# HpWang-whu/YOHO

Measured on AMD Instinct MI355X. Metric: keypoints/sec (5000 kp x60 rot desc+YOHO-O), higher is better.
Workload: dtype fp16x2 split (2^-22-accurate products, fp32 accumulate); 1 GPU

## Files before the change

yoho_amd/csrc/api.hip:

```cpp
#include "common.h"
#include <cstdarg>
#include <cstdio>
#include <cstring>
#include <cstdlib>
#include <cmath>
#include <vector>

namespace yoho {

static thread_local char g_err[512] = "";

void set_error(const char* fmt, ...) {
    va_list ap;
    va_start(ap, fmt);
    vsnprintf(g_err, sizeof(g_err), fmt, ap);
    va_end(ap);
}

void clear_error() { g_err[0] = 0; }

int hip_fail(hipError_t e, const char* what, const char* file, int line) {
    set_error("HIP error %d (%s) at %s:%d: %s", (int)e, hipGetErrorString(e), file, line, what);
    return YOHO_EHIP;
}
// ... 297 lines not shown
        const std::vector<int>* lists[3] = {&all, &two, &one};
        for (int cfg = 0; cfg < 3; ++cfg) {
            const std::vector<int>& gl = *lists[cfg];
            int* ug = &unitg[cfg * 64];
            for (size_t k = 0; k < gl.size(); ++k) ug[k] = gl[k];
            for (int tp = 0; tp < 7; ++tp)
                for (int u = 0; u < 32; ++u)
                    for (int gs = 0; gs < 2; ++gs)
                        for (int h = 0; h < 2; ++h) {
                            int g = ug[2 * u + gs];
                            if (g < 0) g = ug[2 * u];
                            int tap = 2 * tp + h;
                            if (tap >= NTAP) tap = 2 * tp;
                            slab4[(cfg * 7 + tp) * 32 + u] |= (g < 0 ? 0 : (int)N[g * NTAP + tap]) << (8 * (2 * gs + h));
                        }
        }
        if ((rc = upload_slot_tables16(slab4.data(), unitg.data(), c->tabs)) || (rc = gconv16_init())) { delete c; return rc; }
    }
    c->gconv_mode = 4;
    c->partII_mode = 2;
    {
        auto is = [](const char* name, const char* val) { const char* e = std::getenv(name); return e && std::strcmp(e, val) == 0; };
        auto num = [](const char* name) { const char* e = std::getenv(name); return e ? std::atoi(e) : 0; };
        c->env.partII_tail_staged = is("YOHO_PARTII_TAIL", "staged");
        c->env.transfer_staged = is("YOHO_TRANSFER", "staged");
        c->env.xf_steal = !is("YOHO_XF_STEAL", "0");
        c->env.nn_splits = num("YOHO_NN_SPLITS");
        c->env.fcgf_f32 = is("YOHO_FCGF", "f32");
        c->env.fcgf_full_maps = is("YOHO_FCGF_MAPS", "full");
        c->env.fcgf_norm_staged = is("YOHO_FCGF_NORM", "staged");
        c->env.fcgf_heads_staged = is("YOHO_FCGF_HEADS", "staged");
        if (const char* e = std::getenv("YOHO_WS_LIMIT_MB")) c->env.ws_limit_mb = std::atoll(e);
        if (is("YOHO_PARTII_L1", "3")) c->env.partII_l1_variant = FG_TILE256_W8;
    }
    if (const char* m = std::getenv("YOHO_FCGF_CELLS")) c->fcgf_cell_sort = std::atoi(m);
    if (const char* m = std::getenv("YOHO_FCGF_SORT")) c->fcgf_parity_sort = std::strcmp(m, "0") == 0 ? 0 : 1;
    if (const char* m = std::getenv("YOHO_FCGF_COORDS")) c->fcgf_hash_coords = std::strcmp(m, "hash") == 0 ? 1 : 0;
    if (const char* m = std::getenv("YOHO_NN")) c->nn_prefilter = std::strcmp(m, "brute") == 0 ? 0 : 1;
    if (const char* m = std::getenv("YOHO_PARTII")) c->partII_mode = std::strcmp(m, "f32") == 0 ? 0 : (std::strcmp(m, "fp16x2") == 0 ? 2 : (std::strcmp(m, "cgemm") == 0 ? 3 : (std::strcmp(m, "cgemm8") == 0 ? 4 : 1)));
    if (const char* m = std::getenv("YOHO_PARTI_CHUNK")) {
        int ck = 0, ns = 1;
        if (std::sscanf(m, "%dx%d", &ck, &ns) >= 1 && ck >= 0 && (ns == 1 || ns == 2)) { c->partI_chunk = (ck + 255) / 256 * 256; c->partI_streams = ns; }
    }
    if (const char* m = std::getenv("YOHO_GCONV")) c->gconv_mode = std::strcmp(m, "f32") == 0 ? 0 : (std::strcmp(m, "bf16x3") == 0 ? 1 : (std::strcmp(m, "fp16x2") == 0 ? 3 : (std::strcmp(m, "fgemm") == 0 ? 4 : (std::strcmp(m, "fgemm256") == 0 ? 5 : (std::strcmp(m, "fgemm128") == 0 ? 6 : (std::strcmp(m, "fgemm8") == 0 ? 7 : 2))))));
    c->fb = new FourierBasis();
    if ((rc = build_fourier(N, P, *c->fb))) { delete c->fb; delete c; return rc; }
    {
        std::vector<float> fpad(2 * 64 * 64, 0.f);
        for (int s = 0; s < G; ++s)
            for (int g = 0; g < G; ++g) {
                fpad[s * 64 + g] = (float)c->fb->F[s * G + g];
                fpad[64 * 64 + g * 64 + s] = (float)c->fb->F[s * G + g];
            }
        if ((rc = upload(fpad.data(), fpad.size() * sizeof(float), (void**)&c->dFpad)) || (rc = gft_init()) || (rc = fgemm_init()) || (rc = gft16_init())) { delete c->fb; delete c; return rc; }
        std::vector<unsigned short> f16;
        build_gft16_frags(*c->fb, f16);
        if ((rc = upload(f16.data(), f16.size() * sizeof(unsigned short), &c->dF16))) { delete c->fb; delete c; return rc; }
        hipDeviceProp_t prop;
        if (hipGetDeviceProperties(&prop, device) == hipSuccess && prop.multiProcessorCount > 0) c->nCU = prop.multiProcessorCount;
    }
    HIPCHK(hipMalloc((void**)&c->d_rflag, 4 * sizeof(int)));
    HIPCHK(hipMemset(c->d_rflag, 0, 4 * sizeof(int)));
    HIPCHK(hipMalloc((void**)&c->d_amax, 12 * sizeof(unsigned)));
    HIPCHK(hipMemset(c->d_amax, 0, 12 * sizeof(unsigned)));
    {
        for (int g = 0; g < G; ++g) c->cone_slot_of[g] = -1;
// ... 292 lines not shown
    auto mark = [&](int i) { if (prof) (void)hipEventRecord(c->ev[i], s); };
    const Layer* L = c->p1;
    if (prof) { c->ev_chunks = 1; (void)hipEventRecord(c->ev_pass[0], s); }
    mark(0);
    if ((rc = launch_pack_partI(x, B, nT, bS, s))) return rc;
    if ((rc = launch_gft(0, bS, bX, c->dFpad, nullptr, nullptr, nT, 4, s))) return rc;
    mark(1);
    if ((rc = launch_gconvf(L[0], bX, nT, nullptr, bH0, 0, s))) return rc;
    mark(2);
    if ((rc = launch_gft(2, bH0, bA, c->dFpad, L[0].bn_s, L[0].bn_t, nT, 32, s))) return rc;
    mark(3);
    if ((rc = launch_gconvf(L[1], bA, nT, nullptr, bM, 0, s))) return rc;
    mark(4);
    if ((rc = launch_gft(2, bM, bM, c->dFpad, L[1].bn_s, L[1].bn_t, nT, 64, s))) return rc;
    mark(5);
    if ((rc = launch_gconvf(L[2], bM, nT, bH0, bA, EPI_RES, s))) return rc;
    mark(6);
    if ((rc = launch_gft(2, bA, bA, c->dFpad, L[2].bn_s, L[2].bn_t, nT, 32, s))) return rc;
    mark(7);
    if ((rc = launch_gconvf(L[3], bA, nT, nullptr, bY, 0, s))) return rc;
    mark(8);
    if ((rc = launch_gft(1, bY, bYs, c->dFpad, nullptr, nullptr, nT, 4, s))) return rc;
    mark(10);
    if ((rc = launch_finalize_partI(bYs, x, B, eqv, inv, inv_np, 0, s))) return rc;
    mark(9);
    if (prof) (void)hipEventRecord(c->ev_pass[1], s);
    return 0;
}

struct PartIGBufs {
    float *bH0, *bA, *bM, *bY, *bYs;
    char *bP32, *bP256, *bP512;
};
static void partI_G_layout(Arena& ar, int B, PartIGBufs& b) {
    const int nT = (B + TILE - 1) / TILE;
    const int kppad = (B + 255) / 256 * 256;
    const size_t nX = (size_t)nT * 4, n256 = (size_t)nT * 32, n512 = (size_t)nT * 64;
    b.bH0 = ar.take<float>(n256 * CHUNK_FLOATS);
    b.bA = ar.take<float>(n256 * CHUNK_FLOATS);
    b.bM = ar.take<float>(n512 * CHUNK_FLOATS);
    b.bY = ar.take<float>(nX * CHUNK_FLOATS);
    b.bYs = ar.take<float>(nX * CHUNK_FLOATS);
    b.bP32 = ar.take<char>(fgemm_planes_bytes(kppad, 32));
    b.bP256 = ar.take<char>(fgemm_planes_bytes(kppad, 256));
    b.bP512 = ar.take<char>(fgemm_planes_bytes(kppad, 512));
}
static size_t partI_G_ws_bytes(int B) {
    Arena measure;
    PartIGBufs b;
    partI_G_layout(measure, B, b);
    return (measure.off + 4095) / 4096 * 4096;
}

static int partI_passG_chunk(yoho_ctx* c, char* ws, size_t slice, int evbase, const float* x, int B, float* eqv, float* inv, float* inv_np, hipStream_t s,
                             const float* x1, int B0, int slot) {
    const FGemmBlocking gv = c->gconv_mode == 5 ? FG_TILE256_W4 : (c->gconv_mode == 6 ? FG_TILE128 : FG_TILE256_W8);
    const int nT = (B + TILE - 1) / TILE;
    const int kppad = (B + 255) / 256 * 256;
    int rc;
    Arena ar{ws, 0, slice};
    PartIGBufs b;
    partI_G_layout(ar, B, b);
    if (ar.over) { set_error("internal: PartI chunk of %d keypoints does not fit its workspace slice of %zu bytes", B, slice); return YOHO_EINVAL; }
    float *bH0 = b.bH0, *bA = b.bA, *bM = b.bM, *bY = b.bY, *bYs = b.bYs;
    char *bP32 = b.bP32, *bP256 = b.bP256, *bP512 = b.bP512;
    const bool prof = c->profiling && c->ev_created;
    auto mark = [&](int i) { if (prof) (void)hipEventRecord(c->ev[evbase + i], s); };
    const Layer* L = c->p1;
    mark(0);
    int* rf = c->d_rflag;
    int* xc = c->env.xf_steal ? c->d_xfctr + (size_t)slot * 8 : nullptr;
    unsigned* am = c->gconv_mode == 7 ? c->d_amax + (size_t)slot * 4 : nullptr;
    if (am) HIPCHK(hipMemsetAsync(am, 0, 4 * sizeof(unsigned), s));
    if ((rc = launch_head16(x, B, nT, bP32, kppad, c->dF16, s, x1, B0, rf))) return rc;
    mark(1);
    if ((rc = launch_fgemm(L[0], bP32, kppad, nT, nullptr, bH0, 0, s, rf, gv))) return rc;
    mark(2);
    if ((rc = launch_gft16(bH0, nullptr, bP256, kppad, c->dF16, L[0].bn_s, L[0].bn_t, nT, 32, c->nCU, s, 0, rf, gv, xc, am))) return rc;
    mark(3);
    if ((rc = launch_fgemm(L[1], bP256, kppad, nT, nullptr, bM, 0, s, rf, gv, am))) return rc;
    mark(4);
    if ((rc = launch_gft16(bM, nullptr, bP512, kppad, c->dF16, L[1].bn_s, L[1].bn_t, nT, 64, c->nCU, s, 0, rf, gv, xc ? xc + 2 : nullptr, am ? am + 1 : nullptr))) return rc;
    mark(5);
    if ((rc = launch_fgemm(L[2], bP512, kppad, nT, bH0, bA, EPI_RES, s, rf, gv, am ? am + 1 : nullptr))) return rc;
    mark(6);
    if ((rc = launch_gft16(bA, nullptr, bP256, kppad, c->dF16, L[2].bn_s, L[2].bn_t, nT, 32, c->nCU, s, 0, rf, gv, xc ? xc + 4 : nullptr))) return rc;
    mark(7);
    if ((rc = launch_fgemm(L[3], bP256, kppad, nT, nullptr, bY, 0, s, rf, gv))) return rc;
    mark(8);
    if ((rc = launch_gft16(bY, bYs, nullptr, kppad, c->dF16, nullptr, nullptr, nT, 4, c->nCU, s, B, rf))) return rc;
    mark(10);
    if ((rc = launch_finalize_partI(bYs, x, B, eqv, inv, inv_np, 2, s, x1, B0))) return rc;
    mark(9);
    return 0;
}

static int partI_passG(yoho_ctx* c, const float* x, int B, float* eqv, float* inv, float* inv_np, hipStream_t s, const float* x1 = nullptr,
                       int B0 = 0) {
    for (int i = 0; i < 4; ++i) if (!c->p1[i].wpg) { set_error("irrep-GEMM weights missing"); return YOHO_ENOWEIGHTS; }
    const int chunk = c->partI_chunk > 0 ? c->partI_chunk : B;
    const int nch = (B + chunk - 1) / chunk;
    const int nstr = (nch > 1 && c->partI_streams == 2) ? 2 : 1;
    const size_t slice = partI_G_ws_bytes(nch > 1 ? chunk : B);
    int rc;
    static const char* dbg = experiment_env("YOHO_PARTI_DEBUG");
    if ((rc = ensure_ws(c, slice * (size_t)((dbg && std::strstr(dbg, "ownslice")) ? nch : nstr), s))) return rc;
    const bool prof = c->profiling && c->ev_created;
    if (prof) {
        if ((rc = ensure_events(c, nch))) return rc;
        c->ev_chunks = nch;
        (void)hipEventRecord(c->ev_pass[0], s);
    }
    if (nstr == 2) {
        if (!c->side_stream) {
            HIPCHK(hipStreamCreateWithFlags(&c->side_stream, hipStreamNonBlocking));
            HIPCHK(hipEventCreateWithFlags(&c->ev_fork, hipEventDisableTiming));
            HIPCHK(hipEventCreateWithFlags(&c->ev_join, hipEventDisableTiming));
        }
        HIPCHK(hipEventRecord(c->ev_fork, s));
        HIPCHK(hipStreamWaitEvent(c->side_stream, c->ev_fork, 0));
    }
    const bool dbg_serial = dbg && std::strstr(dbg, "serial"), dbg_side = dbg && std::strstr(dbg, "sideonly");
    const bool dbg_own = dbg && std::strstr(dbg, "ownslice");
    for (int k = 0; k < nch; ++k) {
        const int off = k * chunk, n = B - off < chunk ? B - off : chunk;
        const float *xc, *x1c = nullptr;
        int B0c = 0;
        if (x1 && off >= B0) xc = x1 + (size_t)(off - B0) * F * G;
        else {
            xc = x + (size_t)off * F * G;
            if (x1 && off + n > B0) { x1c = x1; B0c = B0 - off; }
        }
        const bool on_side = nstr == 2 && ((k & 1) || dbg_side);
        hipStream_t sk = on_side ? c->side_stream : s;
        char* ws = (char*)c->ws.p + (dbg_own ? slice * (size_t)k : (on_side ? slice : 0));
        if ((rc = partI_passG_chunk(c, ws, slice, k * EV_PER_PASS, xc, n, eqv + (size_t)off * F * G, inv ? inv + (size_t)off * F : nullptr,
// ... 402 lines not shown
```

yoho_amd/csrc/common.h:

```cpp
#pragma once
#include <hip/hip_runtime.h>
#include <stdint.h>
#include <stddef.h>
#include <initializer_list>
#include "yoho_hip.h"
#include "arena.h"

namespace yoho {

constexpr int G = 60;
constexpr int NTAP = 13;
constexpr int F = 32;
constexpr int TILE = 32;
constexpr int SLAB_FLOATS = 2 * TILE * 4;
constexpr int CHUNK_FLOATS = G * SLAB_FLOATS;

void set_error(const char* fmt, ...);
void clear_error();
inline bool yoho_misaligned(std::initializer_list<const void*> ps, unsigned mask) {
    for (const void* p : ps) if ((reinterpret_cast<uintptr_t>(p) & mask) != 0) return true;
    return false;
}
#define YOHO_NEED_ALIGNED(fn, mask, ...)                                                                                  \
    do {                                                                                                                  \
// ... 107 lines not shown
void fgemm_plane_offsets(int kppad, int cin, long long* off);
int pack_fgemm_weights(const FourierBasis& fb, const float* W, int cin, int cout, std::vector<unsigned short>& out, float* descale,
                       std::vector<unsigned short>* out8 = nullptr);
int pack_cgemm_weights(const float* W, int cin, int cout, int ntaps, std::vector<unsigned short>& out, float* descale, std::vector<unsigned short>& out8);
int cgemm_init();
int launch_cgemm(const Layer& L, const char* Bstages, int nslot, const unsigned char* slot, const unsigned char* outg, int nT32, int nTiles16,
                 char* out, hipStream_t s, int* rflag, const unsigned* amax);
int launch_gft16_invg(const float* in, float* res0, char* planesG, const int* slot_of, int nslot, const void* Ffrag, const float* bn_s,
                      const float* bn_t, int nTiles, int C8, int nCU, hipStream_t s, int* rflag, unsigned* amax);
int launch_fgemm(const Layer& L, const char* Bplanes, int kppad, int nT32, const float* res, float* out, int flags, hipStream_t s,
                 int* rflag = nullptr, FGemmBlocking blocking = FG_TILE128, const unsigned* amax = nullptr);
void build_gft16_frags(const FourierBasis& fb, std::vector<unsigned short>& out);
int gconv_layer(yoho_ctx* c, const float* x, int B, int cin, int cout, const float* W, const float* bias, int transpose, float* y,
                hipStream_t s);
int bn_stats(const float* x, int B, int C, float* mean, float* var, hipStream_t s);
int bn_relu_apply(const float* x, int B, int C, const float* scale, const float* shift, float* y, hipStream_t s);
int bn_relu_apply_sub(const float* x, int B, int C, const float* mean, const float* scale, const float* beta, float* y, hipStream_t s);
int bn_relu_backward(const float* x, const float* y, const float* dy, int B, int C, const float* gamma, const float* mean, const float* rstd,
                     int batch_stats, float* dx, float* dgamma, float* dbeta, hipStream_t s);
int gconv_wgrad(yoho_ctx* c, const float* x, const float* dy, int B, int cin, int cout, float* dW, float* db, hipStream_t s);
struct FcgfNet;
int fcgf_load(FcgfNet** out, const yoho_fcgf_config* cfg, const float* const* t, int ntensors, bool f32_kernels);
void fcgf_free(FcgfNet* n);
int fcgf_forward(yoho_ctx* ctx, const FcgfNet* net, const int* coords0, int n0, const int* off_host, int nb, float* out, hipStream_t s);
int fcgf_voxelize(yoho_ctx* ctx, const double* pts, int n, const double* R_host, double voxel, int64_t* sel, int* coords, float* pts_sel,
                  int* count_host, hipStream_t s);
int fcgf_rotate_select(const double* pts, const double* R_host, const int64_t* sel, int m, float* out, hipStream_t s);
int fcgf_voxelize_batch(yoho_ctx* ctx, const double* pts, int n, const double* R_host, int nb, double voxel, int64_t* sel, int* coords,
                        float* pts_sel, int* counts_host, hipStream_t s);
int launch_cone1(const Layer& L, const char* X, int nTiles32, int nTiles16, const float* res, float* out, const int* n0, hipStream_t s, float* part = nullptr);
int gft16_init();
int launch_gft16(const float* in, float* out32, char* planes, int kppad, const void* Ffrag, const float* bn_s, const float* bn_t, int nTiles,
                 int C8, int nCU, hipStream_t s, int B = 0, int* rflag = nullptr, int variant = 2, int* ctr = nullptr, unsigned* amax = nullptr);
int launch_gft16_invp(const float* in, float* res0, char* planes16, int nTiles16, const void* Ffrag, const float* bn_s, const float* bn_t,
                      int nTiles, int C8, int nCU, hipStream_t s, int* rflag = nullptr);
int launch_head2(const float* s0, const float* s1, const float* s2, const float* s3, const int64_t* pre_idx, const int* P, const float* bn_s,
                 const float* bn_t, int M, int nTiles, char* planes, int kppad, const void* Ffrag, hipStream_t s,
                 const int64_t* const* ridx = nullptr, int istride = 1, int* rflag = nullptr);
int launch_head16(const float* x, int B, int nTiles, char* planes, int kppad, const void* Ffrag, hipStream_t s, const float* x1 = nullptr,
                  int B0 = 0, int* rflag = nullptr);
int launch_gconvf(const Layer& L, const float* X, int nTiles, const float* res, float* out, int flags, hipStream_t s);
int launch_gft(int mode, const float* in, float* out, const float* Fpad, const float* bn_s, const float* bn_t, int nTiles, int C8, hipStream_t s);
int upload_slot_tables16(const int* slab4_h, const int* unitg_h, SlotTables& t);
int gconv16_init();
int launch_gconv16(const Layer& L, const char* X, int nTiles, const float* res, float* out_raw, char* out_act, int flags, hipStream_t s,
                   int cfg = 0, float* out_raw32 = nullptr, float* out_act32 = nullptr, int npl = 3, int* rflag = nullptr);
int launch_pack16_partII(const float* s0, const float* s1, const float* s2, const float* s3, const int64_t* pre_idx, const int* P,
                         const float* bn_s, const float* bn_t, int M, int nTiles16, char* out, hipStream_t s, int npl = 3, int* rflag = nullptr);
int launch_pack16_partI(const float* x, int B, int nTiles, char* out, hipStream_t s, int npl = 3, int* rflag = nullptr);
int launch_group_mean_np(const float* eqv, int B, float* out, hipStream_t s);
int launch_pack_partII(const float* s0, const float* s1, const float* s2, const float* s3, const int64_t* pre_idx,
                       const int* P, const float* bn_s, const float* bn_t, int M, int nTiles, float* out, hipStream_t s);
int launch_quat_norm(const float* y, int M, float* quat, hipStream_t s);

struct MfArgs {
    const float* a; const float* b;
    int Na, Nb;
    float* na2; float* nb2;
    _Float16* a16; _Float16* b16;
    unsigned* rowmin; unsigned* colmin;
    unsigned long long* keysA; unsigned long long* keysB;
    unsigned* maxn2;
    int* bad;
    int tilesPer;
    unsigned long long* cand;
    unsigned* ncand; unsigned cap;
// ... 25 lines not shown
inline const char* experiment_env(const char* name) {
#ifdef YOHO_EXPERIMENTS
    return std::getenv(name);
#else
    (void)name;
    return nullptr;
#endif
}

struct PhaseProf {
    static constexpr int NCAT = 16;
    bool on = false;
    std::vector<hipEvent_t> pool;
    size_t used = 0;
    struct Span { int cat; hipEvent_t a, b; };
    std::vector<Span> spans;
    int open_cat = -1;
    hipEvent_t open_ev = nullptr;
    double flops[NCAT] = {0};
    double launches[NCAT] = {0};
};

}

struct yoho_env_switches {
    bool partII_tail_staged = false;
    bool transfer_staged = false;
    bool xf_steal = true;
    int nn_splits = 0;
    bool fcgf_f32 = false;
    bool fcgf_full_maps = false;
    bool fcgf_norm_staged = false;
    bool fcgf_heads_staged = false;
    yoho::FGemmBlocking partII_l1_variant = yoho::FG_TILE128;
    long long ws_limit_mb = 0;
};

struct yoho_ctx {
    int device = 0;
    yoho_env_switches env;
    float* dR32 = nullptr;
    double* dR64 = nullptr;
    int* dN = nullptr;
    int* dP = nullptr;
    unsigned* dPq = nullptr;
    uint8_t hN[60 * 13];
    uint8_t hP[60 * 60];
    float hR[60 * 9];
    bool has_partI = false, has_partII = false;
    yoho::Layer p1[4];
    yoho::Layer p2[6];
    float *p2_init_bn_s = nullptr, *p2_init_bn_t = nullptr;
    int partII_mode = 2;
    int cone_nslot = 0;
    int cone_slot_of[60];
    unsigned char cone_slot[13 * 13];
    unsigned char cone_outg[13];
    int gconv_mode = 4;
    yoho::FourierBasis* fb = nullptr;
    float* dFpad = nullptr;
    void* dF16 = nullptr;
    yoho::FcgfNet* fcgf = nullptr;
    int tap_inv[13] = {0};
    int* d_tap_inv = nullptr;
    int nCU = 256;
    yoho::SlotTables tabs;
// ... 64 lines not shown
```

yoho_amd/csrc/gft16.hip:

```cpp
#include <hip/hip_runtime.h>
#include <cstdlib>
#include <type_traits>
#include <vector>
#include <cmath>
#include <cstring>

#include "common.h"

namespace yoho {

typedef float floatx16 __attribute__((ext_vector_type(16)));
typedef float floatx2 __attribute__((ext_vector_type(2)));
typedef float floatx4 __attribute__((ext_vector_type(4)));
typedef unsigned uintx4 __attribute__((ext_vector_type(4)));
typedef _Float16 halfx8 __attribute__((ext_vector_type(8)));
typedef _Float16 halfx2 __attribute__((ext_vector_type(2)));
typedef const __attribute__((address_space(1))) void* gptr_t;
typedef __attribute__((address_space(3))) void* lptr_t;

constexpr int GB = 65536;
constexpr int G16_LDS = 2 * GB + 1024;
constexpr int G16X_MAXC = 512;
constexpr int G16X_LDS = G16_LDS + 2 * G16X_MAXC * 4;
constexpr float F_SCALE = 1024.f;

struct Gft16Args {
    const float* in;
    float* out32;
    char* planes;
    const uintx4* Ffrag;
    const float* bn_s;
    const float* bn_t;
    int nChunks, C8, B;
    float* res0;
    int nTiles16;
    long long qbase[G];
    int qstride[G];
    int* rflag;
    int drain;
    int* ctr;
// ... 442 lines not shown
        lds_barrier();
        char* dst0 = a.planes + (size_t)(c8 >> 2) * 32768 + (c8 & 3) * 4096 + (tile32 & 7) * 512;
        const int nt = tile32 >> 3;
#pragma unroll
        for (int i = 0; i < 8; ++i) {
            const int idx = i * 512 + tid;
            if (idx < 2 * G * 32) {
                const int pl = idx >= 1920 ? 1 : 0, rem = idx - pl * 1920;
                const int q = rem >> 5, kpp = rem & 31;
                const char* sp = cur + pl * 30720 + q * 512 + kpp * 8;
                uint2 c03, c47;
                asm volatile("ds_read_b64 %0, %2\n\tds_read_b64 %1, %2 offset:256\n\ts_waitcnt lgkmcnt(0)"
                             : "=&v"(c03), "=&v"(c47) : "v"((unsigned)(size_t)sp) : "memory");
                *reinterpret_cast<uintx4*>(dst0 + qb[q] + (long long)nt * qs[q] + kpp * 16 + pl * 16384) = uintx4{c03.x, c03.y, c47.x, c47.y};
            }
        }
        chunk = next;
        if (!steal) nxt = next + gridDim.x;
    }
    note_range_bits(a.rflag, top);
    if (a.amax) {
        unsigned t = top;
#pragma unroll
        for (int o = 32; o >= 1; o >>= 1) t = max(t, (unsigned)__shfl_xor((int)t, o));
        if (lane == 0) atomicMax(a.amax, t);
    }
    if (steal && tid == 0) {
        __builtin_amdgcn_s_waitcnt(0x0F70);
        const int done = __hip_atomic_fetch_add(a.ctr + 1, 1, __ATOMIC_ACQ_REL, __HIP_MEMORY_SCOPE_AGENT);
        if (done == (int)gridDim.x - 1) {
            __hip_atomic_store(a.ctr, 0, __ATOMIC_RELAXED, __HIP_MEMORY_SCOPE_AGENT);
            __hip_atomic_store(a.ctr + 1, 0, __ATOMIC_RELEASE, __HIP_MEMORY_SCOPE_AGENT);
        }
    }
}

static inline unsigned short hbits(float x) {
    const _Float16 h = (_Float16)x;
    unsigned short u;
    std::memcpy(&u, &h, 2);
    return u;
}

void build_gft16_frags(const FourierBasis& fb, std::vector<unsigned short>& out) {
    out.assign((size_t)3 * 2 * 4 * 2 * 64 * 8, 0);
    auto Fv = [&](int q, int g) -> float { return (q < G && g < G) ? (float)fb.F[q * G + g] : 0.f; };
    for (int mat = 0; mat < 3; ++mat)
        for (int rb = 0; rb < 2; ++rb)
            for (int kb = 0; kb < 4; ++kb)
                for (int lane = 0; lane < 64; ++lane)
                    for (int e = 0; e < 8; ++e) {
                        const int i = lane & 31, kg = lane >> 5;
                        float v;
                        if (mat == 0) {
                            const int g = 32 * rb + i, q = 16 * kb + 8 * kg + e;
                            v = Fv(q, g);
                        } else if (mat == 1) {
                            const int q = 32 * rb + i;
                            const int g = 32 * (kb >> 1) + (e & 3) + 8 * (2 * (kb & 1) + (e >> 2)) + 4 * kg;
                            v = Fv(q, g);
                        } else {
                            const int q = 32 * rb + i, g = 16 * kb + 8 * kg + e;
                            v = Fv(q, g);
                        }
                        v *= F_SCALE;
                        const _Float16 hi = (_Float16)v;
                        const size_t base = ((((size_t)mat * 2 + rb) * 4 + kb) * 2) * 512 + lane * 8 + e;
                        out[base] = hbits(v);
                        out[base + 512] = hbits(v - (float)hi);
                    }
}

int gft16_init() {
    HIPCHK(hipFuncSetAttribute(reinterpret_cast<const void*>(&gft16_kernel<G16_ACT32>), hipFuncAttributeMaxDynamicSharedMemorySize, G16_LDS));
    HIPCHK(hipFuncSetAttribute(reinterpret_cast<const void*>(&gft16_kernel<G16_ACTP>), hipFuncAttributeMaxDynamicSharedMemorySize, G16_LDS));
    HIPCHK(hipFuncSetAttribute(reinterpret_cast<const void*>(&gft16_kernel<G16_INV>), hipFuncAttributeMaxDynamicSharedMemorySize, G16_LDS));
    HIPCHK(hipFuncSetAttribute(reinterpret_cast<const void*>(&gft16_kernel<G16_INVP>), hipFuncAttributeMaxDynamicSharedMemorySize, G16_LDS));
    HIPCHK(hipFuncSetAttribute(reinterpret_cast<const void*>(&gft16_kernel<G16_INVG>), hipFuncAttributeMaxDynamicSharedMemorySize, G16_LDS));
    HIPCHK(hipFuncSetAttribute(reinterpret_cast<const void*>(&gft16x_kernel), hipFuncAttributeMaxDynamicSharedMemorySize, G16X_LDS));
    return 0;
}

static void fill_qtables(int kppad, int cin, long long* qbase, int* qstride) {
    int qi[G * 4];
    long long off[NIR_ORD];
    fgemm_qinfo(qi);
    fgemm_plane_offsets(kppad, cin, off);
    for (int q = 0; q < G; ++q) {
        const int t = qi[q * 4], m = qi[q * 4 + 1], j = qi[q * 4 + 2], d = qi[q * 4 + 3];
        const long long KS = d * cin / 32;
        qstride[q] = (int)(KS * 32768);
        qbase[q] = off[t] + ((long long)j * (kppad / 256) * KS + (long long)m * cin / 32) * 32768;
    }
}

int launch_gft16(const float* in, float* out32, char* planes, int kppad, const void* Ffrag, const float* bn_s, const float* bn_t, int nTiles,
                 int C8, int nCU, hipStream_t s, int B, int* rflag, int variant, int* ctr, unsigned* amax) {
    Gft16Args a;
    a.B = B; a.res0 = nullptr; a.nTiles16 = 0; a.rflag = rflag; a.amax = amax;
    a.ctr = ctr;
    a.in = in; a.out32 = out32; a.planes = planes; a.Ffrag = reinterpret_cast<const uintx4*>(Ffrag); a.bn_s = bn_s; a.bn_t = bn_t;
    a.nChunks = nTiles * C8; a.C8 = C8;
    static const int dbg_drain = [] { const char* e = experiment_env("YOHO_PARTI_DEBUG"); return (e && std::strstr(e, "drain")) ? 1 : 0; }();
    static const int dbg_xf1 = [] { const char* e = experiment_env("YOHO_PARTI_DEBUG"); return (e && std::strstr(e, "xf1")) ? 1 : 0; }();
    static const int dbg_ldnt = [] { const char* e = experiment_env("YOHO_PARTI_DEBUG"); return (e && std::strstr(e, "ldnt")) ? 2 : 0; }();
    a.drain = dbg_drain | dbg_ldnt;
    if (dbg_xf1) variant = 1;
    if (planes) {
        fill_qtables(kppad, C8 * 8, a.qbase, a.qstride);
    } else {
        for (int q = 0; q < G; ++q) { a.qbase[q] = 0; a.qstride[q] = 0; }
    }
    static const int gmult = [] { const char* e = experiment_env("YOHO_PARTI_DEBUG"); const char* q = e ? std::strstr(e, "xfgrid") : nullptr; return q ? std::atoi(q + 6) : 1; }();
    const int want = nCU * (gmult > 0 ? gmult : 1);
    const int grid = a.nChunks < want ? a.nChunks : want;
    if (grid == 0) return 0;
    if (a.nChunks <= 2 * grid) a.ctr = nullptr;
    if (planes && variant != 1 && a.C8 * 8 <= G16X_MAXC) hipLaunchKernelGGL(gft16x_kernel, dim3(grid), dim3(512), G16X_LDS, s, a);
    else if (planes) hipLaunchKernelGGL(gft16_kernel<G16_ACTP>, dim3(grid), dim3(256), G16_LDS, s, a);
    else if (bn_s) hipLaunchKernelGGL(gft16_kernel<G16_ACT32>, dim3(grid), dim3(256), G16_LDS, s, a);
    else hipLaunchKernelGGL(gft16_kernel<G16_INV>, dim3(grid), dim3(256), G16_LDS, s, a);
    HIPCHK(hipGetLastError());
    return 0;
}

struct Head16Args {
    const float* x;
    const float* x1;
    int B0;
    char* planes;
    const uintx4* Ffrag;
    int B, nTiles;
    long long qbase[G];
    int qstride[G];
    int* rflag;
};

__global__ __launch_bounds__(256, 1) void head16_kernel(Head16Args a) {
    __shared__ long long qb[G];
    __shared__ int qs[G];
    const int tid = threadIdx.x, lane = tid & 63;
    const int w = __builtin_amdgcn_readfirstlane(tid >> 6);
    const int Lp = lane & 31, kg = lane >> 5;
    if (tid < G) { qb[tid] = a.qbase[tid]; qs[tid] = a.qstride[tid]; }
    __syncthreads();
    const int tile32 = blockIdx.x;
    const int kp = tile32 * TILE + Lp;
    unsigned top = 0u;
    uintx4 A[2][4][2];
#pragma unroll
    for (int rb = 0; rb < 2; ++rb)
#pragma unroll
        for (int kb = 0; kb < 4; ++kb)
#pragma unroll
            for (int pl = 0; pl < 2; ++pl) A[rb][kb][pl] = a.Ffrag[(((2 * 2 + rb) * 4 + kb) * 2 + pl) * 64 + lane];

    floatx16 acc[8][2];
#pragma unroll
// ... 263 lines not shown
```

yoho_amd/csrc/layout.hip:

```cpp
#include "common.h"

namespace yoho {

__device__ __forceinline__ size_t iidx(int tile, int C8, int c, int g, int kp) {
    return ((((size_t)tile * C8 + (c >> 3)) * G + g) * 2 + ((c >> 2) & 1)) * (TILE * 4) + kp * 4 + (c & 3);
}

__global__ __launch_bounds__(256) void pack_partI_kernel(const float* __restrict__ x, int B, float* __restrict__ out) {
    __shared__ float lds[CHUNK_FLOATS];
    const int tile = blockIdx.x >> 2, c8 = blockIdx.x & 3;
    for (int i = threadIdx.x; i < TILE * 8 * G; i += 256) {
        const int kp = i / (8 * G);
        const int r = i - kp * (8 * G);
        const int cl = r / G, g = r - cl * G;
        const int b = tile * TILE + kp;
        const float v = b < B ? x[(size_t)b * (F * G) + (c8 * 8 + cl) * G + g] : 0.f;
        lds[(g * 2 + (cl >> 2)) * (TILE * 4) + kp * 4 + (cl & 3)] = v;
    }
    __syncthreads();
    float4* o = reinterpret_cast<float4*>(out + ((size_t)tile * 4 + c8) * CHUNK_FLOATS);
    const float4* l = reinterpret_cast<const float4*>(lds);
    for (int i = threadIdx.x; i < CHUNK_FLOATS / 4; i += 256) o[i] = l[i];
}

int launch_pack_partI(const float* x, int B, int nTiles, float* out, hipStream_t s) {
    hipLaunchKernelGGL(pack_partI_kernel, dim3(nTiles * 4), dim3(256), 0, s, x, B, out);
    HIPCHK(hipGetLastError());
    return 0;
}

__device__ __forceinline__ float np_pairwise_mean60(const float* v) {
    float r[8];
#pragma unroll
    for (int j = 0; j < 8; ++j) r[j] = v[j];
#pragma unroll
    for (int b = 1; b < 7; ++b)
#pragma unroll
        for (int j = 0; j < 8; ++j) r[j] = __fadd_rn(r[j], v[8 * b + j]);
    float s = __fadd_rn(__fadd_rn(__fadd_rn(r[0], r[1]), __fadd_rn(r[2], r[3])),
                        __fadd_rn(__fadd_rn(r[4], r[5]), __fadd_rn(r[6], r[7])));
#pragma unroll
    for (int j = 56; j < 60; ++j) s = __fadd_rn(s, v[j]);
    return __fdiv_rn(s, 60.0f);
}

__device__ __forceinline__ size_t iidx16(int tile, int C8, int c, int g, int kp) {
    return (((size_t)tile * C8 + (c >> 3)) * G + g) * 128 + kp * 8 + (c & 7);
}

__global__ __launch_bounds__(64) void finalize_partI_kernel(const float* __restrict__ y, const float* __restrict__ x, int B,
                                                            float* __restrict__ eqv, float* __restrict__ inv,
                                                            float* __restrict__ inv_np, int layout16, const float* __restrict__ x1, int B0) {
    __shared__ float e[F * G];
    __shared__ float rn[G];
    const int b = blockIdx.x;
    const int lane = threadIdx.x;
    const int tw = layout16 == 1 ? 16 : TILE;
    const int tile = b / tw, kp = b - tile * tw;
    const float* xb = (x1 && b >= B0) ? x1 + (size_t)(b - B0) * (F * G) : x + (size_t)b * (F * G);
    for (int i = lane; i < F * G; i += 64) {
        const int c = i / G, g = i - c * G;
        e[i] = y[layout16 == 2 ? (size_t)b * (F * G) + i : (layout16 ? iidx16(tile, 4, c, g, kp) : iidx(tile, 4, c, g, kp))] + xb[i];
    }
    __syncthreads();
    if (lane < G) {
        float s = 0.f;
        for (int c = 0; c < F; ++c) { const float v = e[c * G + lane]; s += v * v; }
        rn[lane] = fmaxf(sqrtf(s), 1e-4f);
    }
    if (lane < F && inv != nullptr) {
        float s = 0.f;
        for (int g = 0; g < G; ++g) s += e[lane * G + g];
        const float m = s / 60.0f;
        float n2 = m * m;
        for (int o = 16; o >= 1; o >>= 1) n2 += __shfl_xor(n2, o, 32);
        inv[(size_t)b * F + lane] = m / fmaxf(sqrtf(n2), 1e-4f);
    }
    __syncthreads();
    float* eb = eqv + (size_t)b * (F * G);
    for (int i = lane; i < F * G; i += 64) {
        const int g = i % G;
        const float v = e[i] / rn[g];
        e[i] = v;
        eb[i] = v;
    }
    if (inv_np != nullptr) {
        __syncthreads();
        if (lane < F) inv_np[(size_t)b * F + lane] = np_pairwise_mean60(e + lane * G);
    }
}

int launch_finalize_partI(const float* y, const float* x, int B, float* eqv, float* inv, float* inv_np, int layout16, hipStream_t s,
                          const float* x1, int B0) {
    hipLaunchKernelGGL(finalize_partI_kernel, dim3(B), dim3(64), 0, s, y, x, B, eqv, inv, inv_np, layout16, x1, B0);
    HIPCHK(hipGetLastError());
    return 0;
}

__global__ __launch_bounds__(256) void group_mean_np_kernel(const float* __restrict__ eqv, int rows, float* __restrict__ out) {
    const int r = blockIdx.x * 256 + threadIdx.x;
    if (r >= rows) return;
    float v[G];
    const float4* p = reinterpret_cast<const float4*>(eqv + (size_t)r * G);
#pragma unroll
    for (int i = 0; i < G / 4; ++i) {
        const float4 t = p[i];
        v[4 * i] = t.x; v[4 * i + 1] = t.y; v[4 * i + 2] = t.z; v[4 * i + 3] = t.w;
    }
    out[r] = np_pairwise_mean60(v);
}

int launch_group_mean_np(const float* eqv, int B, float* out, hipStream_t s) {
    const int rows = B * F;
    hipLaunchKernelGGL(group_mean_np_kernel, dim3((rows + 255) / 256), dim3(256), 0, s, eqv, rows, out);
    HIPCHK(hipGetLastError());
// ... 64 lines not shown
```

Baseline: 1.893 million keypoints/s.

## Fuse final inverse group FFT with PartI finalize into one tail kernel

Adds a gtail16 kernel that runs the last inverse group transform (fp16x2 split MFMA) and the PartI finalize (residual add, channel norm, invariant means, eqv write) in one launch, keeping the transformed features in LDS. This removes the bYs intermediate buffer round-trip through global memory and one kernel launch. The previous two-kernel path is kept behind YOHO_PARTI_TAIL=staged. The shared tail math moves into a header with contraction disabled so both paths round identically. The fused kernel uses 64KB LDS and only 8 keypoints per block, which may limit occupancy.

```diff
diff --git a/yoho_amd/csrc/api.hip b/yoho_amd/csrc/api.hip
--- a/yoho_amd/csrc/api.hip
+++ b/yoho_amd/csrc/api.hip
@@ -353,6 +353,7 @@
         c->env.fcgf_heads_staged = is("YOHO_FCGF_HEADS", "staged");
         if (const char* e = std::getenv("YOHO_WS_LIMIT_MB")) c->env.ws_limit_mb = std::atoll(e);
         if (is("YOHO_PARTII_L1", "3")) c->env.partII_l1_variant = FG_TILE256_W8;
+        c->env.partI_tail_staged = is("YOHO_PARTI_TAIL", "staged");
     }
     if (const char* m = std::getenv("YOHO_FCGF_CELLS")) c->fcgf_cell_sort = std::atoi(m);
     if (const char* m = std::getenv("YOHO_FCGF_SORT")) c->fcgf_parity_sort = std::strcmp(m, "0") == 0 ? 0 : 1;
@@ -711,7 +712,7 @@
     float *bH0, *bA, *bM, *bY, *bYs;
     char *bP32, *bP256, *bP512;
 };
-static void partI_G_layout(Arena& ar, int B, PartIGBufs& b) {
+static void partI_G_layout(Arena& ar, int B, PartIGBufs& b, bool tail_staged) {
     const int nT = (B + TILE - 1) / TILE;
     const int kppad = (B + 255) / 256 * 256;
     const size_t nX = (size_t)nT * 4, n256 = (size_t)nT * 32, n512 = (size_t)nT * 64;
@@ -719,15 +720,15 @@
     b.bA = ar.take<float>(n256 * CHUNK_FLOATS);
     b.bM = ar.take<float>(n512 * CHUNK_FLOATS);
     b.bY = ar.take<float>(nX * CHUNK_FLOATS);
-    b.bYs = ar.take<float>(nX * CHUNK_FLOATS);
+    b.bYs = tail_staged ? ar.take<float>(nX * CHUNK_FLOATS) : nullptr;
     b.bP32 = ar.take<char>(fgemm_planes_bytes(kppad, 32));
     b.bP256 = ar.take<char>(fgemm_planes_bytes(kppad, 256));
     b.bP512 = ar.take<char>(fgemm_planes_bytes(kppad, 512));
 }
-static size_t partI_G_ws_bytes(int B) {
+static size_t partI_G_ws_bytes(int B, bool tail_staged) {
     Arena measure;
     PartIGBufs b;
-    partI_G_layout(measure, B, b);
+    partI_G_layout(measure, B, b, tail_staged);
     return (measure.off + 4095) / 4096 * 4096;
 }
 
@@ -739,7 +740,7 @@
     int rc;
     Arena ar{ws, 0, slice};
     PartIGBufs b;
-    partI_G_layout(ar, B, b);
+    partI_G_layout(ar, B, b, c->env.partI_tail_staged);
     if (ar.over) { set_error("internal: PartI chunk of %d keypoints does not fit its workspace slice of %zu bytes", B, slice); return YOHO_EINVAL; }
     float *bH0 = b.bH0, *bA = b.bA, *bM = b.bM, *bY = b.bY, *bYs = b.bYs;
     char *bP32 = b.bP32, *bP256 = b.bP256, *bP512 = b.bP512;
@@ -767,9 +768,14 @@
     mark(7);
     if ((rc = launch_fgemm(L[3], bP256, kppad, nT, nullptr, bY, 0, s, rf, gv))) return rc;
     mark(8);
-    if ((rc = launch_gft16(bY, bYs, nullptr, kppad, c->dF16, nullptr, nullptr, nT, 4, c->nCU, s, B, rf))) return rc;
-    mark(10);
-    if ((rc = launch_finalize_partI(bYs, x, B, eqv, inv, inv_np, 2, s, x1, B0))) return rc;
+    if (c->env.partI_tail_staged) {
+        if ((rc = launch_gft16(bY, bYs, nullptr, kppad, c->dF16, nullptr, nullptr, nT, 4, c->nCU, s, B, rf))) return rc;
+        mark(10);
+        if ((rc = launch_finalize_partI(bYs, x, B, eqv, inv, inv_np, 2, s, x1, B0))) return rc;
+    } else {
+        if ((rc = launch_gtail16(bY, x, B, eqv, inv, inv_np, c->dF16, s, x1, B0))) return rc;
+        mark(10);
+    }
     mark(9);
     return 0;
 }
@@ -780,7 +786,7 @@
     const int chunk = c->partI_chunk > 0 ? c->partI_chunk : B;
     const int nch = (B + chunk - 1) / chunk;
     const int nstr = (nch > 1 && c->partI_streams == 2) ? 2 : 1;
-    const size_t slice = partI_G_ws_bytes(nch > 1 ? chunk : B);
+    const size_t slice = partI_G_ws_bytes(nch > 1 ? chunk : B, c->env.partI_tail_staged);
     int rc;
     static const char* dbg = experiment_env("YOHO_PARTI_DEBUG");
     if ((rc = ensure_ws(c, slice * (size_t)((dbg && std::strstr(dbg, "ownslice")) ? nch : nstr), s))) return rc;
diff --git a/yoho_amd/csrc/common.h b/yoho_amd/csrc/common.h
--- a/yoho_amd/csrc/common.h
+++ b/yoho_amd/csrc/common.h
@@ -163,6 +163,8 @@
 int gft16_init();
 int launch_gft16(const float* in, float* out32, char* planes, int kppad, const void* Ffrag, const float* bn_s, const float* bn_t, int nTiles,
                  int C8, int nCU, hipStream_t s, int B = 0, int* rflag = nullptr, int variant = 2, int* ctr = nullptr, unsigned* amax = nullptr);
+int launch_gtail16(const float* in, const float* x, int B, float* eqv, float* inv, float* inv_np, const void* Ffrag, hipStream_t s,
+                   const float* x1 = nullptr, int B0 = 0);
 int launch_gft16_invp(const float* in, float* res0, char* planes16, int nTiles16, const void* Ffrag, const float* bn_s, const float* bn_t,
                       int nTiles, int C8, int nCU, hipStream_t s, int* rflag = nullptr);
 int launch_head2(const float* s0, const float* s1, const float* s2, const float* s3, const int64_t* pre_idx, const int* P, const float* bn_s,
@@ -254,6 +256,7 @@
     bool fcgf_full_maps = false;
     bool fcgf_norm_staged = false;
     bool fcgf_heads_staged = false;
+    bool partI_tail_staged = false;
     yoho::FGemmBlocking partII_l1_variant = yoho::FG_TILE128;
     long long ws_limit_mb = 0;
 };
diff --git a/yoho_amd/csrc/gft16.hip b/yoho_amd/csrc/gft16.hip
--- a/yoho_amd/csrc/gft16.hip
+++ b/yoho_amd/csrc/gft16.hip
@@ -6,6 +6,7 @@
 #include <cstring>
 
 #include "common.h"
+#include "partI_tail.h"
 
 namespace yoho {
 
@@ -514,6 +515,150 @@
             __hip_atomic_store(a.ctr, 0, __ATOMIC_RELAXED, __HIP_MEMORY_SCOPE_AGENT);
             __hip_atomic_store(a.ctr + 1, 0, __ATOMIC_RELEASE, __HIP_MEMORY_SCOPE_AGENT);
         }
+    }
+}
+
+constexpr int GT_KP = 8;
+constexpr int GT_LDS = 64 * 1024;
+
+struct GTailArgs {
+    const float* in;
+    const float* x;
+    const float* x1;
+    int B0, B;
+    float* eqv;
+    float* inv;
+    float* inv_np;
+    const uintx4* Ffrag;
+};
+
+__global__ __launch_bounds__(256, 2) void gtail16_kernel(GTailArgs a) {
+    extern __shared__ __attribute__((aligned(16))) char smem[];
+    const int tid = threadIdx.x, lane = tid & 63;
+    const int w = __builtin_amdgcn_readfirstlane(tid >> 6);
+    const int Lp = lane & 31, kg = lane >> 5;
+    const int tile32 = blockIdx.x >> 2, qt = blockIdx.x & 3;
+    const int kp0 = blockIdx.x * GT_KP;
+
+    {
+        const char* src = reinterpret_cast<const char*>(a.in) + (size_t)tile32 * G * 4 * 1024 + (lane >> 4) * 1024 + ((lane >> 3) & 1) * 512 +
+                          qt * 128 + (lane & 7) * 16;
+        for (int q = w; q < G; q += 4) __builtin_amdgcn_global_load_lds((gptr_t)(src + (size_t)q * 4096), (lptr_t)(smem + q * 1024), 16, 0, 0);
+    }
+    reinterpret_cast<uintx4*>(smem + G * 1024)[tid] = uintx4{0u, 0u, 0u, 0u};
+
+    uintx4 A1[2][4][2];
+#pragma unroll
+    for (int rb = 0; rb < 2; ++rb)
+#pragma unroll
+        for (int kb = 0; kb < 4; ++kb)
+#pragma unroll
+            for (int pl = 0; pl < 2; ++pl) A1[rb][kb][pl] = a.Ffrag[(((0 * 2 + rb) * 4 + kb) * 2 + pl) * 64 + lane];
+    asm volatile("s_waitcnt vmcnt(0)" ::: "memory");
+    __syncthreads();
+
+    floatx16 acc[2][2];
+#pragma unroll
+    for (int rb = 0; rb < 2; ++rb)
+#pragma unroll
+        for (int f = 0; f < 2; ++f)
+#pragma unroll
+            for (int r = 0; r < 16; ++r) acc[rb][f][r] = 0.f;
+    const char* colp = smem + w * 256 + Lp * 8 + kg * 8 * 1024;
+#pragma unroll
+    for (int kb = 0; kb < 4; ++kb) {
+        floatx2 v[8];
+#pragma unroll
+        for (int e = 0; e < 8; ++e) v[e] = *reinterpret_cast<const floatx2*>(colp + (kb * 16 + e) * 1024) * HF_ASCALE;
+        uintx4 bh[2], bl[2];
+#pragma unroll
+        for (int p = 0; p < 4; ++p) {
+            unsigned h0, l0, h1, l1;
+            split_pair(v[2 * p].x, v[2 * p + 1].x, h0, l0);
+            split_pair(v[2 * p].y, v[2 * p + 1].y, h1, l1);
+            bh[0][p] = h0; bl[0][p] = l0; bh[1][p] = h1; bl[1][p] = l1;
+        }
+#pragma unroll
+        for (int rb = 0; rb < 2; ++rb)
+#pragma unroll
+            for (int f = 0; f < 2; ++f) acc[rb][f] = mfma_hh(A1[rb][kb][1], bh[f], acc[rb][f]);
+#pragma unroll
+        for (int rb = 0; rb < 2; ++rb)
+#pragma unroll
+            for (int f = 0; f < 2; ++f) acc[rb][f] = mfma_hh(A1[rb][kb][0], bl[f], acc[rb][f]);
+#pragma unroll
+        for (int rb = 0; rb < 2; ++rb)
+#pragma unroll
+            for (int f = 0; f < 2; ++f) acc[rb][f] = mfma_hh(A1[rb][kb][0], bh[f], acc[rb][f]);
+    }
+
+    float* E = reinterpret_cast<float*>(smem);
+    floatx4 xv[15];
+#pragma unroll
+    for (int j = 0; j < 15; ++j) {
+        const int i4 = j * 256 + tid, kl = i4 / (F * G / 4), b = kp0 + kl;
+        const float* xrow = (a.x1 && b >= a.B0) ? a.x1 + (size_t)(b - a.B0) * (F * G) : a.x + (size_t)b * (F * G);
+        xv[j] = b < a.B ? *reinterpret_cast<const floatx4*>(xrow + (i4 - kl * (F * G / 4)) * 4) : floatx4{0.f, 0.f, 0.f, 0.f};
+    }
+    __syncthreads();
+    {
+        const float osc = 1.f / (F_SCALE * HF_ASCALE);
+#pragma unroll
+        for (int f = 0; f < 2; ++f) {
+            const int c = w * 8 + (Lp >> 4) * 4 + 2 * (Lp & 1) + f;
+            float* dst = E + (((Lp & 15) >> 1) * F + c) * G;
+#pragma unroll
+            for (int rb = 0; rb < 2; ++rb)
+#pragma unroll
+                for (int t4 = 0; t4 < 4; ++t4) {
+                    const int g0 = 32 * rb + 8 * t4 + 4 * kg;
+                    floatx4 o;
+                    o.x = acc[rb][f][4 * t4] * osc; o.y = acc[rb][f][4 * t4 + 1] * osc;
+                    o.z = acc[rb][f][4 * t4 + 2] * osc; o.w = acc[rb][f][4 * t4 + 3] * osc;
+                    if (g0 < G) *reinterpret_cast<floatx4*>(dst + g0) = o;
+                }
+        }
+    }
+    __syncthreads();
+#pragma unroll
+    for (int j = 0; j < 15; ++j) {
+        floatx4* p = reinterpret_cast<floatx4*>(E) + j * 256 + tid;
+        const floatx4 y = *p;
+        floatx4 o;
+        o.x = tail_residual(y.x, xv[j].x); o.y = tail_residual(y.y, xv[j].y);
+        o.z = tail_residual(y.z, xv[j].z); o.w = tail_residual(y.w, xv[j].w);
+        *p = o;
+    }
+    __syncthreads();
+    const int bk = kp0 + (tid >> 5);
+    if (a.inv != nullptr) {
+        const float r = tail_inv_normalise(tail_group_mean(E + tid * G));
+        if (bk < a.B) a.inv[(size_t)bk * F + (tid & 31)] = r;
+        __syncthreads();
+    }
+    for (int i = tid; i < GT_KP * G; i += 256) {
+        const int kl = i / G, g = i - kl * G;
+        float* col = E + kl * (F * G) + g;
+        const float rn = tail_channel_norm(col, G);
+        for (int c = 0; c < F; ++c) col[c * G] = tail_normalise(col[c * G], rn);
+    }
+    __syncthreads();
+    if (a.inv_np != nullptr) {
+        float v[G];
+        const floatx4* p = reinterpret_cast<const floatx4*>(E + tid * G);
+#pragma unroll
+        for (int i = 0; i < G / 4; ++i) {
+            const floatx4 t = p[i];
+            v[4 * i] = t.x; v[4 * i + 1] = t.y; v[4 * i + 2] = t.z; v[4 * i + 3] = t.w;
+        }
+        const float r = np_pairwise_mean60(v);
+        if (bk < a.B) a.inv_np[(size_t)bk * F + (tid & 31)] = r;
+    }
+    floatx4* eb = reinterpret_cast<floatx4*>(a.eqv + (size_t)kp0 * (F * G));
+#pragma unroll
+    for (int j = 0; j < 15; ++j) {
+        const int i4 = j * 256 + tid;
+        if (kp0 + i4 / (F * G / 4) < a.B) eb[i4] = reinterpret_cast<const floatx4*>(E)[i4];
     }
 }
 
@@ -560,6 +705,7 @@
     HIPCHK(hipFuncSetAttribute(reinterpret_cast<const void*>(&gft16_kernel<G16_INVP>), hipFuncAttributeMaxDynamicSharedMemorySize, G16_LDS));
     HIPCHK(hipFuncSetAttribute(reinterpret_cast<const void*>(&gft16_kernel<G16_INVG>), hipFuncAttributeMaxDynamicSharedMemorySize, G16_LDS));
     HIPCHK(hipFuncSetAttribute(reinterpret_cast<const void*>(&gft16x_kernel), hipFuncAttributeMaxDynamicSharedMemorySize, G16X_LDS));
+    HIPCHK(hipFuncSetAttribute(reinterpret_cast<const void*>(&gtail16_kernel), hipFuncAttributeMaxDynamicSharedMemorySize, GT_LDS));
     return 0;
 }
 
@@ -606,6 +752,17 @@
     return 0;
 }
 
+int launch_gtail16(const float* in, const float* x, int B, float* eqv, float* inv, float* inv_np, const void* Ffrag, hipStream_t s,
+                   const float* x1, int B0) {
+    GTailArgs a;
+    a.in = in; a.x = x; a.x1 = x1; a.B0 = B0; a.B = B; a.eqv = eqv; a.inv = inv; a.inv_np = inv_np;
+    a.Ffrag = reinterpret_cast<const uintx4*>(Ffrag);
+    if (B <= 0) return 0;
+    hipLaunchKernelGGL(gtail16_kernel, dim3((B + GT_KP - 1) / GT_KP), dim3(256), GT_LDS, s, a);
+    HIPCHK(hipGetLastError());
+    return 0;
+}
+
 struct Head16Args {
     const float* x;
     const float* x1;
diff --git a/yoho_amd/csrc/layout.hip b/yoho_amd/csrc/layout.hip
--- a/yoho_amd/csrc/layout.hip
+++ b/yoho_amd/csrc/layout.hip
@@ -1,4 +1,5 @@
 #include "common.h"
+#include "partI_tail.h"
 
 namespace yoho {
 
@@ -29,21 +30,6 @@
     return 0;
 }
 
-__device__ __forceinline__ float np_pairwise_mean60(const float* v) {
-    float r[8];
-#pragma unroll
-    for (int j = 0; j < 8; ++j) r[j] = v[j];
-#pragma unroll
-    for (int b = 1; b < 7; ++b)
-#pragma unroll
-        for (int j = 0; j < 8; ++j) r[j] = __fadd_rn(r[j], v[8 * b + j]);
-    float s = __fadd_rn(__fadd_rn(__fadd_rn(r[0], r[1]), __fadd_rn(r[2], r[3])),
-                        __fadd_rn(__fadd_rn(r[4], r[5]), __fadd_rn(r[6], r[7])));
-#pragma unroll
-    for (int j = 56; j < 60; ++j) s = __fadd_rn(s, v[j]);
-    return __fdiv_rn(s, 60.0f);
-}
-
 __device__ __forceinline__ size_t iidx16(int tile, int C8, int c, int g, int kp) {
     return (((size_t)tile * C8 + (c >> 3)) * G + g) * 128 + kp * 8 + (c & 7);
 }
@@ -60,27 +46,16 @@
     const float* xb = (x1 && b >= B0) ? x1 + (size_t)(b - B0) * (F * G) : x + (size_t)b * (F * G);
     for (int i = lane; i < F * G; i += 64) {
         const int c = i / G, g = i - c * G;
-        e[i] = y[layout16 == 2 ? (size_t)b * (F * G) + i : (layout16 ? iidx16(tile, 4, c, g, kp) : iidx(tile, 4, c, g, kp))] + xb[i];
+        e[i] = tail_residual(y[layout16 == 2 ? (size_t)b * (F * G) + i : (layout16 ? iidx16(tile, 4, c, g, kp) : iidx(tile, 4, c, g, kp))], xb[i]);
     }
     __syncthreads();
-    if (lane < G) {
-        float s = 0.f;
-        for (int c = 0; c < F; ++c) { const float v = e[c * G + lane]; s += v * v; }
-        rn[lane] = fmaxf(sqrtf(s), 1e-4f);
-    }
-    if (lane < F && inv != nullptr) {
-        float s = 0.f;
-        for (int g = 0; g < G; ++g) s += e[lane * G + g];
-        const float m = s / 60.0f;
-        float n2 = m * m;
-        for (int o = 16; o >= 1; o >>= 1) n2 += __shfl_xor(n2, o, 32);
-        inv[(size_t)b * F + lane] = m / fmaxf(sqrtf(n2), 1e-4f);
-    }
+    if (lane < G) rn[lane] = tail_channel_norm(e + lane, G);
+    if (lane < F && inv != nullptr) inv[(size_t)b * F + lane] = tail_inv_normalise(tail_group_mean(e + lane * G));
     __syncthreads();
     float* eb = eqv + (size_t)b * (F * G);
     for (int i = lane; i < F * G; i += 64) {
         const int g = i % G;
-        const float v = e[i] / rn[g];
+        const float v = tail_normalise(e[i], rn[g]);
         e[i] = v;
         eb[i] = v;
     }
diff --git a/yoho_amd/csrc/partI_tail.h b/yoho_amd/csrc/partI_tail.h
--- /dev/null
+++ b/yoho_amd/csrc/partI_tail.h
@@ -0,0 +1,52 @@
+#pragma once
+#include "common.h"
+
+namespace yoho {
+
+__device__ __forceinline__ float np_pairwise_mean60(const float* v) {
+#pragma clang fp contract(off)
+    float r[8];
+#pragma unroll
+    for (int j = 0; j < 8; ++j) r[j] = v[j];
+#pragma unroll
+    for (int b = 1; b < 7; ++b)
+#pragma unroll
+        for (int j = 0; j < 8; ++j) r[j] = __fadd_rn(r[j], v[8 * b + j]);
+    float s = __fadd_rn(__fadd_rn(__fadd_rn(r[0], r[1]), __fadd_rn(r[2], r[3])),
+                        __fadd_rn(__fadd_rn(r[4], r[5]), __fadd_rn(r[6], r[7])));
+#pragma unroll
+    for (int j = 56; j < 60; ++j) s = __fadd_rn(s, v[j]);
+    return __fdiv_rn(s, 60.0f);
+}
+
+__device__ __forceinline__ float tail_residual(float y, float x) {
+#pragma clang fp contract(off)
+    return y + x;
+}
+
+__device__ __forceinline__ float tail_channel_norm(const float* e, int stride) {
+#pragma clang fp contract(off)
+    float s = 0.f;
+    for (int c = 0; c < F; ++c) { const float v = e[c * stride]; s += v * v; }
+    return fmaxf(sqrtf(s), 1e-4f);
+}
+
+__device__ __forceinline__ float tail_group_mean(const float* e) {
+#pragma clang fp contract(off)
+    float s = 0.f;
+    for (int g = 0; g < G; ++g) s += e[g];
+    return s / 60.0f;
+}
+
+__device__ __forceinline__ float tail_inv_normalise(float m) {
+#pragma clang fp contract(off)
+    float n2 = m * m;
+    for (int o = 16; o >= 1; o >>= 1) n2 += __shfl_xor(n2, o, 32);
+    return m / fmaxf(sqrtf(n2), 1e-4f);
+}
+
+__device__ __forceinline__ float tail_normalise(float v, float rn) {
+    return v / rn;
+}
+
+}
```

Result: no change. 1.905 million keypoints/s, median of 6 (+0.6%).
